# sharonct/CTPA-CLIP

Measured on AMD Instinct MI355X. Metric: CT-report pairs/sec (contrastive step), higher is better.
Workload: dtype bf16

## Files before the change

### ctpa-clip_amd/csrc/gemm256.hip

```cpp
#include "common.h"
#include <string.h>
#include "../../include/ctclip_hip.h"

namespace g256 {

constexpr int BN = 256, BK = 32;
constexpr int EP_LD = 68;
template <int WR> struct Cfg {
  static constexpr int BM = 128 * WR, NTH = 256 * WR;
  static constexpr int ABYTES = BM * BK * 2, BBYTES = BN * BK * 2, STAGE = ABYTES + BBYTES;
  static constexpr int NSTAGE = WR == 2 ? 4 : 3;
  static constexpr int SMEM = NSTAGE * STAGE;
  static constexpr int GA = ABYTES / 16 / NTH, GB = BBYTES / 16 / NTH, G = GA + GB;
};

struct P {
  int64_t M, N, K;
  const u16* A; int64_t lda;
  const u16* B; int64_t ldb;
  void* C; int64_t ldc; int c_f32;
  u16* C2; int64_t ldc2;
  const float* bias;
  const void* R; int64_t ldr; int r_f32;
  float alpha; int act; int accumulate; int split_k;
// ... 624 lines not shown
          bi = x > best ? c : bi;
          second = __builtin_amdgcn_fmed3f(best, second, x);
          best = fmaxf(best, x);
        }
      auto merge = [&](float ob, float os, int oi) {
        const bool take = ob > best || (ob == best && oi < bi);
        second = take ? fmaxf(best, os) : fmaxf(second, ob);
        bi = take ? oi : bi;
        best = take ? ob : best;
      };
      if (GEMM_PERMLANE) {
        { const float ob = xorf<16>(best, lane), os = xorf<16>(second, lane); merge(ob, os, xori<16>(bi, lane)); }
        { const float ob = xorf<32>(best, lane), os = xorf<32>(second, lane); merge(ob, os, xori<32>(bi, lane)); }
      } else {
#pragma unroll
        for (int o = 16; o <= 32; o <<= 1)
          merge(__shfl_xor(best, o, 64), __shfl_xor(second, o, 64), __shfl_xor(bi, o, 64));
      }
      if (g == 0 && rok && wcol0 < p.N) {
        float2* out = (float2*)p.C + bidx * p.sC;
        out[gm * p.ldc + (wcol0 >> 6)] = make_float2(best, __int_as_float((int)(wcol0 + bi)));
        if (p.C2) ((float*)p.C2)[bidx * p.sC2 + gm * p.ldc2 + (wcol0 >> 6)] = second;
      }
      continue;
    }
    if constexpr (MODE == 8) {
      if (fold) {
        const int64_t gr = rok ? gm : p.M - 1;
        const float mu = p.ln_mean[gr], rs = p.ln_rstd[gr];
#pragma unroll
        for (int j = 0; j < 4; ++j)
#pragma unroll
          for (int r = 0; r < 4; ++r) v[j][r] = rs * (v[j][r] - mu * bias[j][r]);
      }
    }
    if constexpr (MODE == 6 || MODE == 8) {
      float qb[4][4];
#pragma unroll
      for (int j = 0; j < 4; ++j)
#pragma unroll
        for (int r = 0; r < 4; ++r) qb[j][r] = bf2f(f2bf(v[j][r]));
      store_row_bf16((u16*)p.C + bidx * p.sC + gm * p.ldc + wcol0, v, g, rok && wcol0 >= p.c_col0, wcol0, p.N);
      if (wcol0 < p.n2) {
        const int d0 = pair_coff(g);
        const float* sp = p.bias + d0 + (MODE == 8 && !fold ? 32 : 0);
        const f32x4 s0v = *(const f32x4*)sp, s1v = *(const f32x4*)(sp + 4);
#pragma unroll
        for (int jp = 0; jp < 2; ++jp) {
          float c8[8];
#pragma unroll
          for (int k = 0; k < 4; ++k) {
            const auto r = __builtin_amdgcn_permlane16_swap(__float_as_uint(qb[2 * jp][k]),
                                                            __float_as_uint(qb[2 * jp + 1][k]), false, false);
            c8[k] = __uint_as_float(r[0]);
            c8[4 + k] = __uint_as_float(r[1]);
          }
          float ss = 0.f;
#pragma unroll
          for (int e = 0; e < 8; ++e) ss += c8[e] * c8[e];
          if (GEMM_PERMLANE) {
            ss += xorf<32>(ss, lane);
            ss += xorf<16>(ss, lane);
          } else {
            ss += __shfl_xor(ss, 32, 64);
            ss += __shfl_xor(ss, 16, 64);
          }
          const float inv = 1.f / fmaxf(sqrtf(ss), 1e-12f);
          float o8[8];
#pragma unroll
          for (int e = 0; e < 4; ++e) { o8[e] = c8[e] * inv * s0v[e]; o8[4 + e] = c8[4 + e] * inv * s1v[e]; }
          const int64_t c0 = wcol0 + 32 * jp + d0;
          if (rok && c0 < p.n2) st16(p.C2 + bidx * p.sC2 + gm * p.ldc2 + c0, pack8(o8));
        }
      }
      continue;
    }
    if constexpr (MODE == 5) {
      float* Cf = (float*)p.C + (int64_t)split * p.M * p.ldc + bidx * p.sC + gm * p.ldc + cl;
#pragma unroll
      for (int j = 0; j < 4; ++j)
        if (rok && cl + 16 * j < p.N) *(f32x4*)(Cf + 16 * j) = f32x4{v[j][0], v[j][1], v[j][2], v[j][3]};
      continue;
    }
    if constexpr (MODE == 2) {
      if constexpr (LDS) {
        const int64_t gm0 = wrow0 + i * 16;
        store_blk_bf16_lds(scr, (u16*)p.C + bidx * p.sC + gm0 * p.ldc + wcol0, p.ldc, gm0, p.M, wcol0, p.N, v, g, m,
                           lane, p.epi_lds == 2);
        float gg[2][4];
#pragma unroll
        for (int j = 0; j < 2; ++j)
#pragma unroll
          for (int r = 0; r < 4; ++r) gg[j][r] = gelu_erf(bf2f(f2bf(v[j + 2][r]))) * bf2f(f2bf(v[j][r]));
        *(u32x4*)(scr + SCR_GOFF + m * SCR_G + pair_coff(g) * 2) = pair_swap(gg[0], gg[1]);
        const int r = lane >> 2, c = (lane & 3) * 8;
        const u32x4 d = *(const u32x4*)(scr + SCR_GOFF + r * SCR_G + c * 2);
        if (gm0 + r < p.M && wcol0 < p.N) {
          if (p.epi_lds == 2) st16_sc1(p.C2 + bidx * p.sC2 + (gm0 + r) * p.ldc2 + (wcol0 >> 1) + c, d);
          else st16(p.C2 + bidx * p.sC2 + (gm0 + r) * p.ldc2 + (wcol0 >> 1) + c, d);
        }
        continue;
      }
      if constexpr (X3) {
        float gg[2][4], gh[2][4], gl[2][4], hv[4][4];
#pragma unroll
        for (int j = 0; j < 2; ++j)
#pragma unroll
          for (int r = 0; r < 4; ++r) {
            float ge, dge;
            gelu_erf_and_grad(v[j + 2][r], ge, dge);
            hv[j][r] = ge;
            hv[j + 2][r] = v[j][r] * dge;
            gg[j][r] = ge * v[j][r];
            gh[j][r] = rh(gg[j][r]);
            gl[j][r] = gg[j][r] - gh[j][r];
          }
        store_row_f16((u16*)p.C + bidx * p.sC + gm * p.ldc + wcol0, hv, g, rok, wcol0, p.N);
        const u32x4 dh = pair_swap_h(gh[0], gh[1]), dl = pair_swap_h(gl[0], gl[1]), db = pair_swap(gg[0], gg[1]);
        if (rok && wcol0 < p.N) {
          const int64_t gc = (wcol0 >> 1) + pair_coff(g);
          st16(p.C2 + bidx * p.sC2 + gm * p.ldc2 + gc, dh);
          st16(p.C3 + gm * p.ldc3 + gc, dl);
          if (p.C4) st16(p.C4 + gm * p.ldc4 + gc, db);
        }
        continue;
      }
      float gg[2][4];
      if constexpr (H16) {
        float hv[4][4];
#pragma unroll
        for (int j = 0; j < 2; ++j)
#pragma unroll
          for (int r = 0; r < 4; ++r) {
            const float xb = rh(v[j][r]);
            float ge, dge;
            gelu_erf_and_grad(rh(v[j + 2][r]), ge, dge);
            hv[j][r] = ge;
            hv[j + 2][r] = xb * dge;
            gg[j][r] = ge * xb;
          }
        store_row_f16((u16*)p.C + bidx * p.sC + gm * p.ldc + wcol0, hv, g, rok && p.C, wcol0, p.N);
      } else {
        store_row_bf16((u16*)p.C + bidx * p.sC + gm * p.ldc + wcol0, v, g, rok, wcol0, p.N, p.epi_lds == 3);
#pragma unroll
        for (int j = 0; j < 2; ++j)
#pragma unroll
          for (int r = 0; r < 4; ++r) gg[j][r] = gelu_erf(bf2f(f2bf(v[j + 2][r]))) * bf2f(f2bf(v[j][r]));
      }
      const u32x4 d = pair_swap(gg[0], gg[1]);
      if (rok && wcol0 < p.N) {
        if (p.epi_lds == 3) st16_sc1(p.C2 + bidx * p.sC2 + gm * p.ldc2 + (wcol0 >> 1) + pair_coff(g), d);
        else st16(p.C2 + bidx * p.sC2 + gm * p.ldc2 + (wcol0 >> 1) + pair_coff(g), d);
      }
      continue;
    }
    if constexpr (MODE != 0) continue;
#pragma unroll
    for (int j = 0; j < 4; ++j)
#pragma unroll
      for (int r = 0; r < 4; ++r) v[j][r] += bias[j][r];
    if (p.R) {
      if (p.r_f32) {
        const float* Rp = (const float*)p.R + bidx * p.sR + gm * p.ldr + cl;
#pragma unroll
        for (int j = 0; j < 4; ++j)
          if (rok && cl + 16 * j < p.N) {
            const f32x4 a = *(const f32x4*)(Rp + 16 * j);
#pragma unroll
            for (int r = 0; r < 4; ++r) v[j][r] += a[r];
          }
      } else {
        const u16* Rp = (const u16*)p.R + bidx * p.sR + gm * p.ldr + cl;
#pragma unroll
        for (int j = 0; j < 4; ++j)
          if (rok && cl + 16 * j < p.N) {
            float rr[4];
            unpack4(*(const uint2*)(Rp + 16 * j), rr);
#pragma unroll
            for (int r = 0; r < 4; ++r) v[j][r] += rr[r];
          }
      }
    }
    if (p.act == 1) {
      if (p.C2) store_row_bf16(p.C2 + bidx * p.sC2 + gm * p.ldc2 + wcol0, v, g, rok, wcol0, p.N);
#pragma unroll
      for (int j = 0; j < 4; ++j)
#pragma unroll
        for (int r = 0; r < 4; ++r) v[j][r] = gelu_erf(v[j][r]);
    }
    if (p.c_f32) {
      float* Cf = (float*)p.C + bidx * p.sC + gm * p.ldc + cl;
#pragma unroll
      for (int j = 0; j < 4; ++j)
        if (rok && cl + 16 * j < p.N) {
          if (p.accumulate) {
            const f32x4 a = *(const f32x4*)(Cf + 16 * j);
#pragma unroll
            for (int r = 0; r < 4; ++r) v[j][r] += a[r];
          }
          *(f32x4*)(Cf + 16 * j) = f32x4{v[j][0], v[j][1], v[j][2], v[j][3]};
        }
    } else {
      u16* Cb = (u16*)p.C + bidx * p.sC + gm * p.ldc + wcol0;
      if (p.accumulate) {
#pragma unroll
        for (int j = 0; j < 4; ++j)
          if (rok && cl + 16 * j < p.N) {
            float rr[4];
            unpack4(*(const uint2*)(Cb + 16 * j + 4 * g), rr);
#pragma unroll
            for (int r = 0; r < 4; ++r) v[j][r] += rr[r];
          }
      }
      if constexpr (LDS) {
        const int64_t gm0 = wrow0 + i * 16;
        store_blk_bf16_lds(scr, (u16*)p.C + bidx * p.sC + gm0 * p.ldc + wcol0, p.ldc, gm0, p.M, wcol0, p.N, v, g, m,
                           lane, p.epi_lds == 2);
      } else {
        store_row_bf16(Cb, v, g, rok, wcol0, p.N, p.epi_lds == 3);
      }
    }
    if (p.C2 && p.act == 0) {
      if constexpr (LDS) {
        const int64_t gm0 = wrow0 + i * 16;
        store_blk_bf16_lds(scr, p.C2 + bidx * p.sC2 + gm0 * p.ldc2 + wcol0, p.ldc2, gm0, p.M, wcol0, p.N, v, g, m,
                           lane, p.epi_lds == 2);
      } else {
        store_row_bf16(p.C2 + bidx * p.sC2 + gm * p.ldc2 + wcol0, v, g, rok, wcol0, p.N, p.epi_lds == 3);
      }
    }
  }
}

#ifndef GEGLU_BWD_LA
#define GEGLU_BWD_LA 1
#endif
__device__ __forceinline__ void epilogue_geglu_bwd(const P& p, f32x4 (&acc)[8][4], int wr, int wc, int lane,
                                                   int64_t m0, int64_t n0, int bidx) {
  const int m = lane & 15, g = lane >> 4;
  const int64_t wrow0 = m0 + wr * 128, wcol0 = n0 + wc * 64, t0 = wcol0 >> 5;
  const int co = pair_coff(g);
  const u16* hb = (const u16*)p.R + bidx * p.sR;
  u16* db = (u16*)p.C + bidx * p.sC;
  constexpr int LA = GEGLU_BWD_LA;
  u32x4 hx[LA + 1][2], hg[LA + 1][2];
  auto load = [&](int i, int b) {
    const int64_t gm = wrow0 + i * 16 + m;
#pragma unroll
    for (int jp = 0; jp < 2; ++jp) {
      const int64_t t = t0 + jp;
      if (gm < p.M && t * 32 < p.N) {
        const u16* hp = hb + gm * p.ldr + t * 64 + co;
        hx[b][jp] = *(const u32x4*)hp;
        hg[b][jp] = *(const u32x4*)(hp + 32);
      } else {
        hx[b][jp] = make_uint4(0, 0, 0, 0);
        hg[b][jp] = make_uint4(0, 0, 0, 0);
      }
    }
  };
#pragma unroll
  for (int i = 0; i < LA; ++i) load(i, i);
#pragma unroll
  for (int i = 0; i < 8; ++i) {
    const int b = i % (LA + 1);
    if (i + LA < 8) load(i + LA, (i + LA) % (LA + 1));
    const int64_t gm = wrow0 + i * 16 + m;
#pragma unroll
    for (int jp = 0; jp < 2; ++jp) {
      float v0[4], v1[4];
#pragma unroll
      for (int r = 0; r < 4; ++r) { v0[r] = acc[i][2 * jp][r] * p.alpha; v1[r] = acc[i][2 * jp + 1][r] * p.alpha; }
      float d[8], x[8], gt[8], ox[8], og[8];
      unpack8(pair_swap(v0, v1), d);
      if (p.h16) {
        unpack8h(hx[b][jp], x);
        unpack8h(hg[b][jp], gt);
#pragma unroll
        for (int k = 0; k < 8; ++k) {
          ox[k] = d[k] * x[k];
          og[k] = d[k] * gt[k];
        }
      } else {
        unpack8(hx[b][jp], x);
        unpack8(hg[b][jp], gt);
#pragma unroll
        for (int k = 0; k < 8; ++k) {
          float ge, dge;
          gelu_erf_and_grad(gt[k], ge, dge);
          ox[k] = d[k] * ge;
          og[k] = d[k] * x[k] * dge;
        }
      }
      const int64_t t = t0 + jp;
      if (gm < p.M && t * 32 < p.N) {
        u16* dp = db + gm * p.ldc + t * 64 + co;
        st16(dp, pack8(ox));
        st16(dp + 32, pack8(og));
      }
    }
  }
}

typedef __attribute__((address_space(1))) unsigned long long gu64;
typedef __attribute__((address_space(1))) int gi32;
constexpr int LN_ST = p8::SMEM_P;
constexpr int LN_FIN = LN_ST + 2 * 128 * 4 * 8;
constexpr int SMEM_LN = LN_FIN + 256 * 8;
constexpr unsigned LN_SPIN_LIMIT = 1u << 21;

__device__ __forceinline__ void chan(float& m, float& M2, float mb, float M2b, float half_n) {
  const float d = m - mb;
  M2 = (M2 + M2b) + d * d * half_n;
  m = 0.5f * (m + mb);
}

template <int MODE>
__device__ __forceinline__ void epilogue_ln(const P& p, f32x4 (&acc)[8][4], char* smem, int w, int wr, int wc,
                                            int lane, int64_t m0, int64_t n0) {
  float* cs = (float*)(smem + p8::TILEB + w * (32 * EP_LD * 4));
  float2* st = (float2*)(smem + LN_ST);
  float2* fin = (float2*)(smem + LN_FIN);
  const int tx = (int)(n0 >> 8);
  const int64_t wrow0 = m0 + wr * 128, wcol0 = n0 + wc * 64;
  const int cc = (lane & 7) * 8, rl = lane >> 3;
  const int64_t gn = wcol0 + cc;
  float gam[8], bet[8];
  {
    const f32x4 a = *(const f32x4*)(p.ln_gamma + gn), b = *(const f32x4*)(p.ln_gamma + gn + 4);
    f32x4 c = f32x4{0.f, 0.f, 0.f, 0.f}, d = c;
    if (MODE == 6 && p.ln_beta) { c = *(const f32x4*)(p.ln_beta + gn); d = *(const f32x4*)(p.ln_beta + gn + 4); }
#pragma unroll
    for (int j = 0; j < 4; ++j) { gam[j] = a[j]; gam[4 + j] = b[j]; bet[j] = c[j]; bet[4 + j] = d[j]; }
  }
  f32x4 b0 = f32x4{0.f, 0.f, 0.f, 0.f}, b1 = b0;
  if (MODE == 6 && p.bias) { b0 = *(const f32x4*)(p.bias + gn); b1 = *(const f32x4*)(p.bias + gn + 4); }
  float keep[4][4][8];
  float pg[8], pb[8];
#pragma unroll
  for (int j = 0; j < 8; ++j) { pg[j] = 0.f; pb[j] = 0.f; }

#pragma unroll
  for (int quarter = 0; quarter < 4; ++quarter) {
    __builtin_amdgcn_sched_barrier(0);
#pragma unroll
    for (int i = 0; i < 2; ++i)
#pragma unroll
      for (int j = 0; j < 4; ++j)
#pragma unroll
        for (int r = 0; r < 4; ++r)
          cs[(i * 16 + (lane >> 4) * 4 + r) * EP_LD + j * 16 + (lane & 15)] = acc[quarter * 2 + i][j][r];
    __builtin_amdgcn_s_waitcnt(0xC07F);
    const int64_t rbase = wrow0 + quarter * 32;
    if constexpr (MODE == 6) {
      f32x4 ra[4], rb[4];
#pragma unroll
      for (int it = 0; it < 4; ++it) {
        const float* Rp = (const float*)p.R + (rbase + it * 8 + rl) * p.ldr + gn;
        ra[it] = *(const f32x4*)Rp;
        rb[it] = *(const f32x4*)(Rp + 4);
      }
#pragma unroll
      for (int it = 0; it < 4; ++it) {
        const f32x4 lo = *(const f32x4*)(cs + (it * 8 + rl) * EP_LD + cc);
        const f32x4 hi = *(const f32x4*)(cs + (it * 8 + rl) * EP_LD + cc + 4);
#pragma unroll
        for (int j = 0; j < 4; ++j) {
          keep[quarter][it][j] = lo[j] * p.alpha + b0[j] + ra[it][j];
          keep[quarter][it][4 + j] = hi[j] * p.alpha + b1[j] + rb[it][j];
        }
      }
#pragma unroll
      for (int it = 0; it < 4; ++it) {
        const float* v = keep[quarter][it];
        float* Cf = (float*)p.C + (rbase + it * 8 + rl) * p.ldc + gn;
        *(f32x4*)Cf = f32x4{v[0], v[1], v[2], v[3]};
        *(f32x4*)(Cf + 4) = f32x4{v[4], v[5], v[6], v[7]};
      }
      if (p.C2) {
#pragma unroll
        for (int it = 0; it < 4; ++it) *(u32x4*)(p.C2 + (rbase + it * 8 + rl) * p.ldc2 + gn) = pack8(keep[quarter][it]);
      }
#pragma unroll
      for (int it = 0; it < 4; ++it) {
        const float* v = keep[quarter][it];
        float m = 0.f;
#pragma unroll
        for (int j = 0; j < 8; ++j) m += v[j];
        m *= 0.125f;
        float M2 = 0.f;
#pragma unroll
        for (int j = 0; j < 8; ++j) { const float d = v[j] - m; M2 += d * d; }
#pragma unroll
        for (int o = 1; o <= 4; o <<= 1) chan(m, M2, __shfl_xor(m, o, 64), __shfl_xor(M2, o, 64), 4.f * o);
        if ((lane & 7) == 0) st[(wr * 128 + quarter * 32 + it * 8 + rl) * 4 + wc] = make_float2(m, M2);
      }
    } else {
      float mu[4], rs[4];
      u32x4 kx[4];
#pragma unroll
      for (int it = 0; it < 4; ++it) {
        const int64_t row = rbase + it * 8 + rl;
        kx[it] = *(const u32x4*)(p.ln_x + row * p.ln_ldx + gn);
        mu[it] = p.ln_mean[row];
        rs[it] = p.ln_rstd[row];
      }
#pragma unroll
      for (int it = 0; it < 4; ++it) {
        const f32x4 lo = *(const f32x4*)(cs + (it * 8 + rl) * EP_LD + cc);
        const f32x4 hi = *(const f32x4*)(cs + (it * 8 + rl) * EP_LD + cc + 4);
        float d[8];
#pragma unroll
        for (int j = 0; j < 4; ++j) { d[j] = lo[j] * p.alpha; d[4 + j] = hi[j] * p.alpha; }
        const u32x4 kd = pack8(d);
        *(u32x4*)(p.C2 + (rbase + it * 8 + rl) * p.ldc2 + gn) = kd;
        float dy[8], xv[8];
        unpack8(kd, dy);
        unpack8(kx[it], xv);
        float s1 = 0.f, s2 = 0.f;
#pragma unroll
        for (int j = 0; j < 8; ++j) {
          const float xh = (xv[j] - mu[it]) * rs[it];
          const float g = dy[j] * gam[j];
          s1 += g;
          s2 += g * xh;
        }
#pragma unroll
        for (int o = 1; o <= 4; o <<= 1) { s1 += __shfl_xor(s1, o, 64); s2 += __shfl_xor(s2, o, 64); }
        if ((lane & 7) == 0) st[(wr * 128 + quarter * 32 + it * 8 + rl) * 4 + wc] = make_float2(s1, s2);
      }
    }
    __builtin_amdgcn_s_waitcnt(0xC07F);
  }
  __syncthreads();
  if (wc == 0) {
    gu64* X = (gu64*)p.xchg;
    const unsigned long long tag = (unsigned long long)p.epoch << 32;
    float a0[2], a1[2];
#pragma unroll
    for (int h = 0; h < 2; ++h) {
      const int r = lane + 64 * h;
      const float2 s0 = st[(wr * 128 + r) * 4 + 0], s1 = st[(wr * 128 + r) * 4 + 1];
      const float2 s2 = st[(wr * 128 + r) * 4 + 2], s3 = st[(wr * 128 + r) * 4 + 3];
      if constexpr (MODE == 6) {
        float m = s0.x, M2 = s0.y, mm = s2.x, MM = s2.y;
        chan(m, M2, s1.x, s1.y, 32.f);
        chan(mm, MM, s3.x, s3.y, 32.f);
        chan(m, M2, mm, MM, 64.f);
        a0[h] = m;
        a1[h] = M2;
      } else {
        a0[h] = (s0.x + s1.x) + (s2.x + s3.x);
        a1[h] = (s0.y + s1.y) + (s2.y + s3.y);
      }
      gu64* g = X + ((int64_t)tx * p.M + wrow0 + r) * 2;
      if (!(p.ln_debug && tx == 1 && m0 == 0)) {
        __hip_atomic_store(g, tag | __float_as_uint(a0[h]), __ATOMIC_RELAXED, __HIP_MEMORY_SCOPE_AGENT);
        __hip_atomic_store(g + 1, tag | __float_as_uint(a1[h]), __ATOMIC_RELAXED, __HIP_MEMORY_SCOPE_AGENT);
      }
    }
    const gu64* Y = X + (int64_t)(1 - tx) * p.M * 2;
    unsigned long long q[2][2];
    for (unsigned spins = 0;; ++spins) {
      bool ok = true;
#pragma unroll
      for (int h = 0; h < 2; ++h)
#pragma unroll
        for (int k = 0; k < 2; ++k) {
          q[h][k] = __hip_atomic_load(Y + (wrow0 + lane + 64 * h) * 2 + k, __ATOMIC_RELAXED, __HIP_MEMORY_SCOPE_AGENT);
          ok = ok && (unsigned)(q[h][k] >> 32) == p.epoch;
        }
      if (__all(ok)) break;
      if (spins >= p.spin_limit) {
        if (lane == 0 && p.status) __hip_atomic_store((gi32*)p.status, 1, __ATOMIC_RELAXED, __HIP_MEMORY_SCOPE_AGENT);
        break;
      }
      __builtin_amdgcn_s_sleep(1);
    }
#pragma unroll
    for (int h = 0; h < 2; ++h) {
      const int r = lane + 64 * h;
      const float o0 = __uint_as_float((unsigned)q[h][0]), o1 = __uint_as_float((unsigned)q[h][1]);
      float2 f;
      if constexpr (MODE == 6) {
        float m = a0[h], M2 = a1[h];
        chan(m, M2, o0, o1, 128.f);
        const float rstd = rsqrtf(M2 * (1.f / 512.f) + p.ln_eps);
        f = make_float2(m, rstd);
        if (tx == 0) {
          p.ln_mean[wrow0 + r] = m;
          p.ln_rstd[wrow0 + r] = rstd;
        }
      } else {
        f = make_float2((a0[h] + o0) * (1.f / 512.f), (a1[h] + o1) * (1.f / 512.f));
      }
      fin[wr * 128 + r] = f;
    }
  }
  __syncthreads();
  const u16* lx = p.ln_x;
  u16* lc2 = p.C2;
  const float* lmean = p.ln_mean;
  const float* lrstd = p.ln_rstd;
  int64_t frow0 = wrow0 + rl, fcol = gn;
  asm volatile("" : "+v"(frow0), "+v"(fcol));
#pragma unroll
  for (int quarter = 0; quarter < 4; ++quarter) {
    __builtin_amdgcn_sched_barrier(0);
    const int64_t rbase = frow0 - rl + quarter * 32;
    if constexpr (MODE == 6) {
#pragma unroll
      for (int it = 0; it < 4; ++it) {
        const float2 f = fin[wr * 128 + quarter * 32 + it * 8 + rl];
        float o[8];
#pragma unroll
        for (int j = 0; j < 8; ++j) o[j] = (keep[quarter][it][j] - f.x) * f.y * gam[j] + bet[j];
        if (p.ln_y) *(u32x4*)(p.ln_y + (rbase + it * 8 + rl) * p.ln_ldy + gn) = pack8(o);
        if (p.ln_y16) *(u32x4*)(p.ln_y16 + (rbase + it * 8 + rl) * p.ln_ldy + gn) = pack8h(o);
      }
    } else {
#pragma unroll
      for (int half = 0; half < 2; ++half) {
        __builtin_amdgcn_sched_barrier(0);
        f32x4 ra[2], rb[2];
        float mu[2], rs[2];
        u32x4 kx[2], kd[2];
        const int r0 = (int)frow0 + quarter * 32 + half * 16, c0 = (int)fcol;
#pragma unroll
        for (int it = 0; it < 2; ++it) {
          const int row = r0 + it * 8;
          kx[it] = *(const u32x4*)(lx + (row * (int)p.ln_ldx + c0));
          kd[it] = *(const u32x4*)(lc2 + (row * (int)p.ldc2 + c0));
          const float* Rp = (const float*)p.R + (row * (int)p.ldr + c0);
          ra[it] = *(const f32x4*)Rp;
          rb[it] = *(const f32x4*)(Rp + 4);
          mu[it] = lmean[row];
          rs[it] = lrstd[row];
        }
#pragma unroll
        for (int it = 0; it < 2; ++it) {
          const int row = r0 + it * 8;
          const float2 f = fin[wr * 128 + quarter * 32 + half * 16 + it * 8 + rl];
          float dy[8], xv[8], o[8];
          unpack8(kd[it], dy);
          unpack8(kx[it], xv);
#pragma unroll
          for (int j = 0; j < 8; ++j) {
            const float xh = (xv[j] - mu[it]) * rs[it];
            pg[j] += dy[j] * xh;
            pb[j] += dy[j];
            o[j] = rs[it] * (dy[j] * gam[j] - f.x - xh * f.y) + (j < 4 ? ra[it][j] : rb[it][j - 4]);
          }
          float* Cf = (float*)p.C + (row * (int)p.ldc + c0);
          *(f32x4*)Cf = f32x4{o[0], o[1], o[2], o[3]};
          *(f32x4*)(Cf + 4) = f32x4{o[4], o[5], o[6], o[7]};
          *(u32x4*)(lc2 + (row * (int)p.ldc2 + c0)) = pack8(o);
        }
      }
    }
  }
  if constexpr (MODE == 7) {
#pragma unroll
    for (int j = 0; j < 8; ++j)
#pragma unroll
      for (int o = 8; o <= 32; o <<= 1) { pg[j] += __shfl_xor(pg[j], o, 64); pb[j] += __shfl_xor(pb[j], o, 64); }
    if (rl == 0) {
      const int64_t slab = ((m0 >> 7) + wr) * p.N + gn;
      *(f32x4*)(p.ln_pg + slab) = f32x4{pg[0], pg[1], pg[2], pg[3]};
      *(f32x4*)(p.ln_pg + slab + 4) = f32x4{pg[4], pg[5], pg[6], pg[7]};
      if (p.ln_pb) {
        *(f32x4*)(p.ln_pb + slab) = f32x4{pb[0], pb[1], pb[2], pb[3]};
        *(f32x4*)(p.ln_pb + slab + 4) = f32x4{pb[4], pb[5], pb[6], pb[7]};
      }
    }
  }
}

struct Tile {
  int64_t m0, n0, kbeg;
  int nk, split, bidx;
};

template <bool X3 = false>
__device__ __forceinline__ Tile tile_at(const P& p, int lin, int gx, int gy, int ntiles) {
  int id = lin;
  if (ntiles >= 16) {
    const int xcd = lin & 7, q = ntiles >> 3, r = ntiles & 7;
    id = (xcd < r ? xcd * (q + 1) : r * (q + 1) + (xcd - r) * q) + (lin >> 3);
  }
  const int gxy = gx * gy, z = id / gxy, rem = id - z * gxy;
  int ty, tx;
  if (gx >= p.group_gx) {
    const int GM = p.group_gm > 0 ? p.group_gm : 8;
    const int grp = rem / (GM * gx), y0 = grp * GM, gsz = min(gy - y0, GM), r = rem - grp * GM * gx;
    ty = y0 + r % gsz;
    tx = r / gsz;
  } else {
    ty = rem / gx;
    tx = rem - ty * gx;
  }
  Tile t;
  t.split = z % p.split_k;
  t.bidx = z / p.split_k;
  t.m0 = (int64_t)ty * p8::BM;
  t.n0 = (int64_t)tx * p8::BNN;
  t.kbeg = t.split * p.kper;
  const int64_t kend = min(p.K, t.kbeg + p.kper);
  t.nk = (kend > t.kbeg && !(p.debug & 2)) ? (int)((kend - t.kbeg) / p8::BKK) * (X3 ? 3 : 1) : 0;
  return t;
}

#ifdef CTCLIP_GEMM_STAMPS
__device__ unsigned long long g_stamps[256][32][6];
#define STAMP(k, v)                                                                        \
  do {                                                                                     \
    const unsigned long long t_ = (v);                                                     \
    if (threadIdx.x == 0 && tcount < 32) g_stamps[blockIdx.x][tcount][k] = t_;             \
  } while (0)
#else
#define STAMP(k, v) do { } while (0)
#endif

template <bool AK, bool BKC, int EP, bool H16 = false, bool X3 = false>
__global__ __launch_bounds__(512, 1) void gemm8p_kernel(P p) {
  using namespace p8;
  constexpr bool TR = EP >= 0;
  extern __shared__ __attribute__((aligned(16))) char smem[];
  const int lane = threadIdx.x & 63, w = threadIdx.x >> 6, wr = w >> 2, wc = w & 3;
  const int gx = (int)((p.N + BNN - 1) / BNN), gy = (int)((p.M + BM - 1) / BM);
  const int ntiles = gx * gy * p.gz;
  int lin = p.persist ? (int)blockIdx.x : (int)((blockIdx.z * gridDim.y + blockIdx.y) * gridDim.x + blockIdx.x);
  const int lstride = p.persist ? (int)gridDim.x : ntiles;
  if (lin >= ntiles) return;
  Tile T = tile_at<X3>(p, lin, gx, gy, ntiles);
  if (p.stagger > 0 && lin < 256) {
    const int ng = p.stagger >= 1000 ? 4 : 2, u = p.stagger % 1000, grp = (lin >> 3) & (ng - 1);
    for (int s = 0; s < grp * u; ++s) __builtin_amdgcn_s_sleep(32);
  }

  f32x4 acc[8][4];
#pragma unroll
  for (int i = 0; i < 8; ++i)
#pragma unroll
    for (int j = 0; j < 4; ++j) acc[i][j] = f32x4{0.f, 0.f, 0.f, 0.f};
  const int wu = __builtin_amdgcn_readfirstlane(w);
  char* scr = smem + TILEB + (wu < 4 ? A1 : B1) * HALF + (wu & 3) * 4096;

  auto stage_of = [&](const Tile& tl, int which, int t) {
    if (t >= tl.nk) return;
    char* dst = smem + (t & 1) * TILEB + which * HALF;
    int tk = t;
    const u16* Ab = p.A;
    const u16* Bb = p.B;
    if constexpr (X3) {
      tk = (t * 21846) >> 16;
      const int sub = t - 3 * tk;
      if (sub == 2) Ab = p.alo;
      if (sub == 1) Bb = p.blo;
    }
    const int64_t k0 = tl.kbeg + (int64_t)tk * BKK;
    if (which < 2) stage_half<AK, true>(dst, Ab + tl.bidx * p.sA, p.lda, p.M, tl.m0, k0, which, w, lane);
    else stage_half<BKC, false>(dst, Bb + tl.bidx * p.sB, p.ldb, p.N, tl.n0, k0, which - 2, w, lane);
  };
  auto stage = [&](int which, int t) { stage_of(T, which, t); };

  bf16x8 a[4][2], b0[2][2], b1[2][2];

  const int abase = frag_base<AK>(wr * 64, lane), bbase = frag_base<BKC>(wc * 32, lane);
  auto load_frags = [&](int buf, int q) {
    const char* base = smem + buf * TILEB;
    if (q == 0 || q == 2) {
#pragma unroll
      for (int s = 0; s < 2; ++s)
#pragma unroll
        for (int ii = 0; ii < 4; ++ii) a[ii][s] = hfrag<AK>(base, q == 0 ? A0 : A1, abase, ii, s);
    }
    if (q == 0) {
#pragma unroll
      for (int s = 0; s < 2; ++s)
#pragma unroll
        for (int jj = 0; jj < 2; ++jj) b0[jj][s] = hfrag<BKC>(base, B0, bbase, jj, s);
    }
    if (q == 1) {
#pragma unroll
      for (int s = 0; s < 2; ++s)
#pragma unroll
        for (int jj = 0; jj < 2; ++jj) b1[jj][s] = hfrag<BKC>(base, B1, bbase, jj, s);
    }
  };
  auto mma = [&](int q) {
    const int mi = (q == 0 || q == 1) ? 0 : 1;
    const int ni = (q == 1 || q == 2) ? 1 : 0;
    __builtin_amdgcn_s_setprio(1);
#pragma unroll
    for (int s = 0; s < 2; ++s)
#pragma unroll
      for (int ii = 0; ii < 4; ++ii)
#pragma unroll
        for (int jj = 0; jj < 2; ++jj) {
          const bf16x8 bb = ni ? b1[jj][s] : b0[jj][s];
          acc[mi * 4 + ii][ni * 2 + jj] = TR ? mfma16<H16>(bb, a[ii][s], acc[mi * 4 + ii][ni * 2 + jj])
                                             : mfma16<H16>(a[ii][s], bb, acc[mi * 4 + ii][ni * 2 + jj]);
        }
    __builtin_amdgcn_s_setprio(0);
  };
  auto wait_ahead = [&](bool younger_issued) {
    if (younger_issued) asm volatile("s_waitcnt vmcnt(4)" ::: "memory");
    else asm volatile("s_waitcnt vmcnt(0)" ::: "memory");
  };
  auto compute_phase = [&]() {
    bar();
    asm volatile("s_waitcnt lgkmcnt(0)" ::: "memory");
    __builtin_amdgcn_sched_barrier(0);
  };

  stage(A0, 0); stage(A1, 0); stage(B0, 0); stage(B1, 0);
  stage(A0, 1); stage(B0, 1);
  wait_ahead(T.nk > 1);

  int tcount = 0;
  (void)tcount;
  constexpr bool PRE_OK = TR && (EP == 3 || EP == 4 || (EP == 0 && !BKC));
  bool pre = false;
  while (true) {
    const int nk = T.nk;
    STAMP(0, __builtin_amdgcn_s_memtime());
    STAMP(5, __builtin_amdgcn_s_memrealtime());
    bar();
    if (wr == 1) bar();
    for (int i = 0; 2 * i < nk; ++i) {
      if (i == 1) STAMP(2, __builtin_amdgcn_s_memtime());
      const int te = 2 * i, to = 2 * i + 1;
      const int t1 = (PRE_OK && i == 0 && pre) ? nk : to;
#pragma unroll
      for (int q = 0; q < 4; ++q) {
        load_frags(0, q);
        if (q == 0) stage(B1, t1);
        if (q == 1) stage(A1, t1);
        if (q == 2) stage(A0, te + 2);
        if (q == 3) { stage(B0, te + 2); if (to < nk) wait_ahead(te + 2 < nk); }
        compute_phase();
        mma(q);
        bar();
      }
      if (to < nk) {
#pragma unroll
        for (int q = 0; q < 4; ++q) {
          load_frags(1, q);
          if (q == 0) stage(B1, te + 2);
          if (q == 1) stage(A1, te + 2);
          if (q == 2) stage(A0, to + 2);
          if (q == 3) { stage(B0, to + 2); if (te + 2 < nk) wait_ahead(to + 2 < nk); }
          compute_phase();
          mma(q);
          bar();
        }
      }
    }
    if (wr == 0) bar();
    __syncthreads();
    STAMP(3, __builtin_amdgcn_s_memtime());
    lin += lstride;
    const bool more = lin < ntiles;
    if (more) {
      const Tile nx = tile_at<X3>(p, lin, gx, gy, ntiles);
      stage_of(nx, A0, 0); stage_of(nx, A1, 0); stage_of(nx, B0, 0); stage_of(nx, B1, 0);
      if constexpr (TR) { stage_of(nx, A0, 1); stage_of(nx, B0, 1); }
      if constexpr (PRE_OK) {
        if (p.pre1) { stage_of(nx, B1, 1); stage_of(nx, A1, 1); }
      }
    }
    pre = PRE_OK && more && p.pre1;
    if (p.debug & 1) {
#pragma unroll
      for (int i = 0; i < 8; ++i)
#pragma unroll
        for (int j = 0; j < 4; ++j) asm volatile("" ::"v"(acc[i][j]));
    } else if constexpr (EP == 2 || EP == 12) {
      epilogue_t<2, EP == 12, H16, X3>(p, acc, wr, wc, lane, T.m0, T.n0, T.split, T.bidx, scr);
    } else if constexpr (EP == 4) {
      epilogue_geglu_bwd(p, acc, wr, wc, lane, T.m0, T.n0, T.bidx);
    } else if constexpr (EP == 0 || EP == 10) {
      epilogue_t<0, EP == 10>(p, acc, wr, wc, lane, T.m0, T.n0, T.split, T.bidx, scr);
    } else if constexpr (EP == 3) {
      epilogue_t<3>(p, acc, wr, wc, lane, T.m0, T.n0, T.split, T.bidx, scr);
    } else if constexpr (EP == 6) {
      epilogue_t<6>(p, acc, wr, wc, lane, T.m0, T.n0, T.split, T.bidx, scr);
    } else if constexpr (EP == 8) {
      epilogue_t<8>(p, acc, wr, wc, lane, T.m0, T.n0, T.split, T.bidx, scr);
    } else if constexpr (EP == -8) {
      epilogue<-8>(p, acc, smem + TILEB, w, wr, wc, lane, T.m0, T.n0, T.split, T.bidx);
    } else if constexpr (EP == -6 || EP == -7) {
      epilogue_ln<EP == -6 ? 6 : 7>(p, acc, smem, w, wr, wc, lane, T.m0, T.n0);
    } else {
      epilogue<EP == -2 || EP == -3 || EP == -5 ? EP : -1>(p, acc, smem + TILEB, w, wr, wc, lane, T.m0, T.n0, T.split, T.bidx);
    }
    STAMP(4, __builtin_amdgcn_s_memtime());
    ++tcount;
    if (!more) break;
    T = tile_at<X3>(p, lin, gx, gy, ntiles);
#pragma unroll
    for (int i = 0; i < 8; ++i)
#pragma unroll
      for (int j = 0; j < 4; ++j) acc[i][j] = f32x4{0.f, 0.f, 0.f, 0.f};
    if constexpr (!TR) {
      __syncthreads();
      stage(A0, 1); stage(B0, 1);
    }
    wait_ahead(T.nk > 1);
  }
}

static int g_grid_cap = 0;

template <bool AK, bool BKC, int EP, bool H16 = false, bool X3 = false>
int launch8(const P& p, int batch, hipStream_t st) {
  constexpr int smem = EP == -6 || EP == -7 ? SMEM_LN : p8::SMEM_P;
  static bool attr = false;
  if (!attr) {
    (void)hipFuncSetAttribute((const void*)gemm8p_kernel<AK, BKC, EP, H16, X3>,
                              hipFuncAttributeMaxDynamicSharedMemorySize, smem);
    attr = true;
  }
  const int64_t ntiles = cdiv(p.N, p8::BNN) * cdiv(p.M, p8::BM) * (int64_t)p.gz;
  static bool cap_env = false;
  if (!cap_env) {
    const char* e = getenv("CTCLIP_GEMM_GRID_CAP");
    if (e && g_grid_cap == 0) g_grid_cap = atoi(e);
    cap_env = true;
  }
  static int pre1 = -1;
  if (pre1 < 0) { const char* e = getenv("CTCLIP_GEMM_PRE1"); pre1 = e ? atoi(e) != 0 : 1; }
  if (p.persist) {
    const int64_t cap = g_grid_cap > 0 && g_grid_cap < 256 ? g_grid_cap : 256;
    dim3 grid((unsigned)(ntiles < cap ? ntiles : cap));
    P q = p;
    q.pre1 = pre1;
    hipLaunchKernelGGL((gemm8p_kernel<AK, BKC, EP, H16, X3>), grid, dim3(p8::NTH), smem, st, q);
  } else {
    dim3 grid(cdiv(p.N, p8::BNN), cdiv(p.M, p8::BM), batch * p.split_k);
    hipLaunchKernelGGL((gemm8p_kernel<AK, BKC, EP, H16, X3>), grid, dim3(p8::NTH), smem, st, p);
  }
  CT_CHECK_LAUNCH();
  return 0;
}

template <int WR, bool AK, bool BKC>
int launch(const P& p, int batch, hipStream_t st) {
  using C = Cfg<WR>;
  static bool attr = false;
  if (!attr) {
    (void)hipFuncSetAttribute((const void*)gemm256_kernel<WR, AK, BKC>, hipFuncAttributeMaxDynamicSharedMemorySize,
                              C::SMEM);
    attr = true;
  }
  dim3 grid(cdiv(p.N, BN), cdiv(p.M, C::BM), batch * p.split_k);
  hipLaunchKernelGGL((gemm256_kernel<WR, AK, BKC>), grid, dim3(C::NTH), C::SMEM, st, p);
  CT_CHECK_LAUNCH();
  return 0;
}

template <int WR>
int launch_any(const P& p, bool ak, bool bk, int batch, hipStream_t st) {
  if (ak && bk) return launch<WR, true, true>(p, batch, st);
  if (ak) return launch<WR, true, false>(p, batch, st);
  if (bk) return launch<WR, false, true>(p, batch, st);
  return launch<WR, false, false>(p, batch, st);
}

static int g_variant = -1;
static int g_stagger8 = -1;
static int g_persist = -1;
static int g_epi_lds = -1;
int variant() {
  if (g_variant < 0) {
    const char* e = getenv("CTCLIP_GEMM_VARIANT");
    g_variant = e ? atoi(e) : 8;
    if (g_variant != 1 && g_variant != 2) g_variant = 8;
  }
  return g_variant;
}
int tile_rows() { return variant() == 2 ? 2 : 1; }

template <bool AK, bool BKC>
int launch8_ep(const P& p, int batch, hipStream_t st) {
  if (p.act == 4) return launch8<AK, BKC, 4>(p, batch, st);
  if (p.act == 5) return launch8<AK, BKC, 6>(p, batch, st);
  static int tr_f32 = -1;
  if (tr_f32 < 0) { const char* e = getenv("CTCLIP_GEMM_TR_F32"); tr_f32 = e ? atoi(e) != 0 : 0; }
  const bool tr = (tr_f32 || (!p.c_f32 && !p.R)) && p.split_k <= 1 && p.act != 3;
  if (!tr) {
    static int am_tr = -1;
    if (am_tr < 0) { const char* e = getenv("CTCLIP_GEMM_ARGMAX_TR"); am_tr = e ? atoi(e) != 0 : 1; }
    if (p.act == 3 && am_tr && p.split_k <= 1) return launch8<AK, BKC, 3>(p, batch, st);
    if (p.act == 3) return launch8<AK, BKC, -3>(p, batch, st);
    if (p.split_k > 1) return launch8<AK, BKC, -5>(p, batch, st);
    if (p.R && p.r_f32 && p.c_f32 && p.act == 0 && !p.accumulate) return launch8<AK, BKC, -2>(p, batch, st);
    return launch8<AK, BKC, -1>(p, batch, st);
  }
  const bool relay = p.epi_lds == 1 || p.epi_lds == 2;
  if (p.act == 2) return relay ? launch8<AK, BKC, 12>(p, batch, st) : launch8<AK, BKC, 2>(p, batch, st);
  return relay ? launch8<AK, BKC, 10>(p, batch, st) : launch8<AK, BKC, 0>(p, batch, st);
}

int launch8_h16(const P& p, int batch, hipStream_t st) {
  if (p.split_k > 1 || p.act == 4 || p.act == 5 || p.act == 6) return CT_EINVAL;
  if (p.act == 3) return p.x3 ? CT_EINVAL : launch8<true, true, 3, true>(p, batch, st);
  if (p.x3) {
    if (p.act == 2) return launch8<true, true, 2, true, true>(p, batch, st);
    if (!p.c_f32 || p.act != 0) return CT_EINVAL;
    if (p.R && p.r_f32 && !p.accumulate) return launch8<true, true, -2, true, true>(p, batch, st);
    if (p.R) return CT_EINVAL;
    return launch8<true, true, -1, true, true>(p, batch, st);
  }
  const bool tr = !p.c_f32 && !p.R;
  if (p.act == 2) return launch8<true, true, 2, true>(p, batch, st);
  if (tr) return launch8<true, true, 0, true>(p, batch, st);
  if (p.R && p.r_f32 && p.c_f32 && p.act == 0 && !p.accumulate) return launch8<true, true, -2, true>(p, batch, st);
  return launch8<true, true, -1, true>(p, batch, st);
}

template <bool AK>
int launch8_any(const P& p, bool bk, int batch, hipStream_t st) {
  return bk ? launch8_ep<AK, true>(p, batch, st) : launch8_ep<AK, false>(p, batch, st);
}

}

int ctclip_gemm256(const ctclip_gemm_args* a, int split, int batch, void* stream) {
  using namespace g256;
  P p{};
  memset(&p, 0, sizeof(p));
  p.M = a->M; p.N = a->N; p.K = a->K;
  p.A = (const u16*)a->A; p.lda = a->lda;
  p.B = (const u16*)a->B; p.ldb = a->ldb;
  p.C = a->C; p.ldc = a->ldc; p.c_f32 = a->c_f32;
  p.C2 = (u16*)a->C2; p.ldc2 = a->ldc2;
  p.bias = a->bias;
  p.R = a->R; p.ldr = a->ldr; p.r_f32 = a->r_f32;
  p.alpha = a->alpha; p.act = a->act; p.accumulate = a->accumulate; p.split_k = split;
  p.sA = a->sA; p.sB = a->sB; p.sC = a->sC; p.sC2 = a->sC2; p.sR = a->sR;
  p.n2 = a->n2;
  p.fold_cs = nullptr;
  p.nfold = 0;
  p.h16 = a->ab_f16 || a->r_f16;
  p.ln_y16 = nullptr;
  p.x3 = a->A_lo != nullptr;
  p.alo = (const u16*)a->A_lo;
  p.blo = (const u16*)a->B_lo;
  p.C3 = (u16*)a->C3; p.ldc3 = a->ldc3;
  p.C4 = (u16*)a->C4; p.ldc4 = a->ldc4;
  const int kstep = (variant() == 8 || a->act == 4 || a->act == 5) ? p8::BKK : BK;
  p.kper = (a->K / kstep + split - 1) / split * kstep;
  static int dbg = -1, stag = 0;
  if (dbg < 0) {
    const char* e = getenv("CTCLIP_G256_DEBUG");
    dbg = e ? atoi(e) : 0;
    const char* s = getenv("CTCLIP_G256_STAGGER");
    stag = s ? atoi(s) : 0;
  }
  p.debug = dbg;
  if (g_persist < 0) {
    const char* e = getenv("CTCLIP_GEMM_PERSIST");
    g_persist = e ? (atoi(e) != 0) : 1;
  }
  p.gz = batch * split;
  p.persist = g_persist;
  if (g_epi_lds < 0) {
    const char* e = getenv("CTCLIP_EPI_LDS");
    g_epi_lds = e ? std::min(3, std::max(0, atoi(e))) : 0;
  }
  p.epi_lds = g_epi_lds;
  static int ggx = -1;
  if (ggx < 0) { const char* e = getenv("CTCLIP_GEMM_GROUP_GX"); ggx = e ? atoi(e) : 8; }
  p.group_gx = ggx;
  static int ggm = -1;
  if (ggm < 0) { const char* e = getenv("CTCLIP_GEMM_GROUP_GM"); ggm = e ? atoi(e) : 8; }
  p.group_gm = ggm;
  p.stagger = variant() == 8 ? (g_stagger8 >= 0 ? g_stagger8 : (a->act == 4 ? 8 : 0)) : (tile_rows() == 1 ? stag : 0);
  hipStream_t st = (hipStream_t)stream;
  if (a->ab_f16) {
    if (!a->a_kcontig || !a->b_kcontig) return CT_EINVAL;
    p.stagger = 0;
    return launch8_h16(p, batch, st);
  }
  if (variant() == 8 || a->act == 4 || a->act == 5)
    return a->a_kcontig ? launch8_any<true>(p, a->b_kcontig, batch, st) : launch8_any<false>(p, a->b_kcontig, batch, st);
  if (tile_rows() == 2) return launch_any<2>(p, a->a_kcontig, a->b_kcontig, batch, st);
  return launch_any<1>(p, a->a_kcontig, a->b_kcontig, batch, st);
}

extern "C" int ctclip_gemm_ln(const ctclip_gemm_args* a, const ctclip_ln_epilogue* ln, void* stream) {
  using namespace g256;
  if (!a || !ln || (ln->mode != 1 && ln->mode != 2)) return CT_EINVAL;
  if (a->M == 0) return 0;
  CT_REQUIRE(a->N == 512 && a->M > 0 && a->M % 2048 == 0 && a->K > 0 && a->K % 64 == 0, CT_ESHAPE);
  CT_REQUIRE(a->split_k <= 1 && a->batch <= 1 && a->act == 0 && !a->accumulate && a->c_f32 && !a->B2, CT_EINVAL);
  CT_REQUIRE(variant() == 8 && g_persist != 0 && g_grid_cap == 0, CT_EINVAL);
  CT_REQUIRE(aligned16(a->A) && aligned16(a->B) && aligned16(a->C) && a->lda % 8 == 0 && a->ldb % 8 == 0 &&
                 a->ldc % 8 == 0, CT_EALIGN);
  if (a->C2) CT_REQUIRE(aligned16(a->C2) && a->ldc2 % 8 == 0, CT_EALIGN);
  if (a->R) CT_REQUIRE(a->r_f32 && aligned16(a->R) && a->ldr % 8 == 0, CT_EINVAL);
  if (a->bias) CT_REQUIRE(ln->mode == 1 && aligned16(a->bias), CT_EINVAL);
  CT_REQUIRE(ln->gamma && aligned16(ln->gamma) && ln->mean && ln->rstd && ln->xchg && ln->epoch != 0 &&
                 (((uintptr_t)ln->xchg) & 7) == 0, CT_EINVAL);
  {
    const int64_t ldmax = std::max(std::max(a->ldc, a->ldc2), std::max(a->ldr, ln->ldx));
    CT_REQUIRE(a->M * ldmax < ((int64_t)1 << 31), CT_ESHAPE);
  }
  if (ln->mode == 1) {
    CT_REQUIRE(a->R && (ln->Y || ln->Y16) && aligned16(ln->Y) && aligned16(ln->Y16) && ln->ldy % 8 == 0, CT_EINVAL);
    if (ln->beta) CT_REQUIRE(aligned16(ln->beta), CT_EALIGN);
  } else {
    CT_REQUIRE(ln->X && aligned16(ln->X) && ln->ldx % 8 == 0 && ln->part_gamma && !ln->beta && a->C2 && a->R,
               CT_EINVAL);
  }
  P p{};
  memset(&p, 0, sizeof(p));
  p.M = a->M; p.N = a->N; p.K = a->K;
  p.A = (const u16*)a->A; p.lda = a->lda;
  p.B = (const u16*)a->B; p.ldb = a->ldb;
  p.C = a->C; p.ldc = a->ldc; p.c_f32 = 1;
  p.C2 = (u16*)a->C2; p.ldc2 = a->ldc2;
  p.bias = a->bias;
  p.R = a->R; p.ldr = a->ldr; p.r_f32 = 1;
  p.alpha = a->alpha; p.act = 0; p.accumulate = 0; p.split_k = 1;
  p.kper = a->K;
  p.debug = 0;
  p.group_gx = 1 << 30;
  p.stagger = 0;
  p.gz = 1;
  p.persist = 1;
  p.ln_gamma = ln->gamma; p.ln_beta = ln->beta; p.ln_eps = ln->eps;
  p.ln_y = (u16*)ln->Y; p.ln_ldy = ln->ldy;
  p.ln_mean = ln->mean; p.ln_rstd = ln->rstd;
  p.ln_x = (const u16*)ln->X; p.ln_ldx = ln->ldx;
  p.ln_pg = ln->part_gamma; p.ln_pb = ln->part_beta;
  p.xchg = (unsigned long long*)ln->xchg;
  p.epoch = ln->epoch;
  p.status = ln->status;
  p.spin_limit = ln->spin_limit ? ln->spin_limit : LN_SPIN_LIMIT;
  p.ln_debug = ln->debug;
  p.ln_y16 = ln->mode == 1 ? (u16*)ln->Y16 : nullptr;
  hipStream_t st = (hipStream_t)stream;
  if (!a->a_kcontig) return CT_EINVAL;
  if (a->ab_f16) {
    if (ln->mode != 1 || !a->b_kcontig) return CT_EINVAL;
    return launch8<true, true, -6, true>(p, 1, st);
  }
  if (ln->mode == 1) return a->b_kcontig ? launch8<true, true, -6>(p, 1, st) : launch8<true, false, -6>(p, 1, st);
  return a->b_kcontig ? launch8<true, true, -7>(p, 1, st) : launch8<true, false, -7>(p, 1, st);
}

extern "C" int ctclip_gemm_qkv_lnfold(const ctclip_gemm_args* a, const float* mean, const float* rstd,
                                      const float* fold_cs, int32_t nfold, void* stream) {
  return ctclip_gemm_qkv_lnfold2(a, mean, rstd, fold_cs, nfold, 0, stream);
}

extern "C" int ctclip_gemm_qkv_lnfold2(const ctclip_gemm_args* a, const float* mean, const float* rstd,
                                       const float* fold_cs, int32_t nfold, int32_t c_col0, void* stream) {
  using namespace g256;
  if (c_col0 < 0 || c_col0 % 64) return CT_EINVAL;
  if (!a || !mean || !rstd || !fold_cs) return CT_EINVAL;
  if (a->M == 0) return 0;
  CT_REQUIRE(a->M > 0 && a->N % 256 == 0 && a->K > 0 && a->K % 64 == 0, CT_ESHAPE);
  CT_REQUIRE(nfold > 0 && nfold % 256 == 0 && nfold < a->N && a->n2 > nfold && a->n2 % 64 == 0 && a->n2 <= a->N,
             CT_EINVAL);
  CT_REQUIRE(a->a_kcontig && a->b_kcontig && !a->c_f32 && a->C2 && a->bias && !a->R && !a->B2 && a->act == 5 &&
                 a->split_k <= 1 && a->batch <= 1 && !a->accumulate,
             CT_EINVAL);
  CT_REQUIRE(variant() == 8, CT_EINVAL);
  CT_REQUIRE(aligned16(a->A) && aligned16(a->B) && aligned16(a->C) && aligned16(a->C2) && aligned16(a->bias) &&
                 aligned16(fold_cs) && a->lda % 8 == 0 && a->ldb % 8 == 0 && a->ldc % 8 == 0 && a->ldc2 % 8 == 0,
             CT_EALIGN);
  P p{};
  memset(&p, 0, sizeof(p));
  p.M = a->M; p.N = a->N; p.K = a->K;
  p.A = (const u16*)a->A; p.lda = a->lda;
  p.B = (const u16*)a->B; p.ldb = a->ldb;
  p.C = a->C; p.ldc = a->ldc; p.c_f32 = 0;
  p.C2 = (u16*)a->C2; p.ldc2 = a->ldc2;
  p.bias = a->bias;
  p.alpha = a->alpha; p.act = 5; p.split_k = 1;
  p.n2 = a->n2;
  p.kper = a->K;
  p.gz = 1;
  if (g_persist < 0) {
    const char* e = getenv("CTCLIP_GEMM_PERSIST");
    g_persist = e ? (atoi(e) != 0) : 1;
  }
  p.persist = g_persist;
  p.group_gx = 8;
  p.ln_mean = (float*)mean;
  p.ln_rstd = (float*)rstd;
  p.fold_cs = fold_cs;
  p.nfold = nfold;
  p.c_col0 = c_col0;
  if (a->ab_f16) return launch8<true, true, 8, true>(p, 1, (hipStream_t)stream);
  return launch8<true, true, 8>(p, 1, (hipStream_t)stream);
}

extern "C" int ctclip_gemm_lnfold_bwd(const ctclip_gemm_args* a, const void* X, int64_t ldx, const float* c1,
                                      const float* beta, void* stream) {
  using namespace g256;
  if (!a || !X || !c1 || !beta) return CT_EINVAL;
  if (a->M == 0) return 0;
  CT_REQUIRE(a->M > 0 && a->N > 0 && a->N % 8 == 0 && a->K > 0 && a->K % 64 == 0, CT_ESHAPE);
  CT_REQUIRE(a->a_kcontig && a->c_f32 && a->R && a->r_f32 && !a->bias && !a->B2 && a->act == 0 && a->split_k <= 1 &&
                 a->batch <= 1 && !a->accumulate,
             CT_EINVAL);
  CT_REQUIRE(variant() == 8, CT_EINVAL);
  CT_REQUIRE(aligned16(a->A) && aligned16(a->B) && aligned16(a->C) && aligned16(a->R) && aligned16(X) &&
                 a->lda % 8 == 0 && a->ldb % 8 == 0 && a->ldc % 8 == 0 && a->ldr % 8 == 0 && ldx % 8 == 0,
             CT_EALIGN);
  if (a->C2) CT_REQUIRE(aligned16(a->C2) && a->ldc2 % 8 == 0, CT_EALIGN);
  P p{};
  memset(&p, 0, sizeof(p));
  p.M = a->M; p.N = a->N; p.K = a->K;
  p.A = (const u16*)a->A; p.lda = a->lda;
  p.B = (const u16*)a->B; p.ldb = a->ldb;
  p.C = a->C; p.ldc = a->ldc; p.c_f32 = 1;
  p.C2 = (u16*)a->C2; p.ldc2 = a->ldc2;
  p.R = a->R; p.ldr = a->ldr; p.r_f32 = 1;
  p.alpha = a->alpha; p.split_k = 1;
  p.kper = a->K;
  p.gz = 1;
  if (g_persist < 0) {
    const char* e = getenv("CTCLIP_GEMM_PERSIST");
    g_persist = e ? (atoi(e) != 0) : 1;
  }
  p.persist = g_persist;
  p.group_gx = 8;
  p.ln_x = (const u16*)X;
  p.ln_ldx = ldx;
  p.ln_mean = (float*)c1;
  p.ln_rstd = (float*)beta;
  hipStream_t st = (hipStream_t)stream;
  return a->b_kcontig ? launch8<true, true, -8>(p, 1, st) : launch8<true, false, -8>(p, 1, st);
}

extern "C" int ctclip_gemm_set_epi_lds(int v) {
  const int old = g256::g_epi_lds;
  g256::g_epi_lds = v >= 0 && v <= 3 ? v : 0;
  return old;
}

extern "C" int ctclip_gemm_set_stagger(int v) {
  const int old = g256::g_stagger8;
  g256::g_stagger8 = v;
  return old;
}

extern "C" int ctclip_gemm_set_grid_cap(int v) {
  const int old = g256::g_grid_cap;
  g256::g_grid_cap = v > 0 ? v : 0;
  return old;
}

extern "C" int ctclip_gemm_set_persist(int v) {
  const int old = g256::g_persist;
  g256::g_persist = v != 0;
  return old;
}

extern "C" int ctclip_gemm_set_variant(int v) {
  const int old = g256::variant();
  if (v == 1 || v == 2 || v == 8) g256::g_variant = v;
  return old;
}

#ifdef CTCLIP_GEMM_STAMPS
extern "C" int ctclip_gemm_stamps(void* host, int clear) {
  hipError_t e = hipMemcpyFromSymbol(host, HIP_SYMBOL(g256::g_stamps), sizeof(g256::g_stamps), 0, hipMemcpyDeviceToHost);
  if (e == hipSuccess && clear) {
    static unsigned long long zero[256 * 32 * 6];
    e = hipMemcpyToSymbol(HIP_SYMBOL(g256::g_stamps), zero, sizeof(zero), 0, hipMemcpyHostToDevice);
  }
  return (int)e;
}
#endif
```

Measured before the change: 205.9.

## Relay GEGLU backward epilogue through LDS for coalesced row loads and stores

Result: faster. 208.3, median of 6 (+1.2%).

```diff
diff --git a/ctpa-clip_amd/csrc/gemm256.hip b/ctpa-clip_amd/csrc/gemm256.hip
--- a/ctpa-clip_amd/csrc/gemm256.hip
+++ b/ctpa-clip_amd/csrc/gemm256.hip
@@ -950,6 +950,84 @@
   }
 }
 
+#ifndef GEGLU_BWD_ROWS_LA
+#define GEGLU_BWD_ROWS_LA 1
+#endif
+constexpr int GB_STRIP = 16 * 256;
+constexpr int SMEM_GB = 2 * p8::TILEB + 8 * GB_STRIP;
+__device__ __forceinline__ void epilogue_geglu_bwd_rows(const P& p, f32x4 (&acc)[8][4], int wr, int wc, int lane,
+                                                        int64_t m0, int64_t n0, int bidx, char* scr) {
+  const int64_t wrow0 = m0 + wr * 128, wcol0 = n0 + wc * 64, t0 = wcol0 >> 5;
+  if (wcol0 >= p.N) return;
+  asm volatile("" : "+v"(lane));
+  const int m = lane & 15, g = lane >> 4;
+  const int rr = lane >> 4, pc = lane & 15;
+  const bool cok = (t0 + (pc >> 3)) * 32 < p.N;
+  const u16* hb = (const u16*)p.R + bidx * p.sR + t0 * 64 + pc * 8;
+  u16* db = (u16*)p.C + bidx * p.sC + t0 * 64 + pc * 8;
+  const int cx = pair_coff(g) >> 3;
+  constexpr int LA = GEGLU_BWD_ROWS_LA;
+  u32x4 hr[LA][4];
+  auto load = [&](int i, int b) {
+#pragma unroll
+    for (int q = 0; q < 4; ++q) {
+      const int64_t gm = wrow0 + i * 16 + q * 4 + rr;
+      hr[b][q] = (gm < p.M && cok) ? *(const u32x4*)(hb + gm * p.ldr) : make_uint4(0, 0, 0, 0);
+    }
+  };
+#pragma unroll
+  for (int i = 0; i < LA; ++i) load(i, i);
+#pragma unroll
+  for (int i = 0; i < 8; ++i) {
+    const int b = i % LA;
+#pragma unroll
+    for (int q = 0; q < 4; ++q) {
+      const int r = q * 4 + rr;
+      *(u32x4*)(scr + r * 256 + ((pc ^ r) << 4)) = hr[b][q];
+    }
+    if (i + LA < 8) load(i + LA, b);
+#pragma unroll
+    for (int jp = 0; jp < 2; ++jp) {
+      char* sx = scr + m * 256 + (((jp * 8 + cx) ^ m) << 4);
+      char* sg = scr + m * 256 + (((jp * 8 + 4 + cx) ^ m) << 4);
+      const u32x4 hx = *(const u32x4*)sx, hg = *(const u32x4*)sg;
+      float v0[4], v1[4];
+#pragma unroll
+      for (int r = 0; r < 4; ++r) { v0[r] = acc[i][2 * jp][r] * p.alpha; v1[r] = acc[i][2 * jp + 1][r] * p.alpha; }
+      float d[8], x[8], gt[8], ox[8], og[8];
+      unpack8(pair_swap(v0, v1), d);
+      if (p.h16) {
+        unpack8h(hx, x);
+        unpack8h(hg, gt);
+#pragma unroll
+        for (int k = 0; k < 8; ++k) {
+          ox[k] = d[k] * x[k];
+          og[k] = d[k] * gt[k];
+        }
+      } else {
+        unpack8(hx, x);
+        unpack8(hg, gt);
+#pragma unroll
+        for (int k = 0; k < 8; ++k) {
+          float ge, dge;
+          gelu_erf_and_grad(gt[k], ge, dge);
+          ox[k] = d[k] * ge;
+          og[k] = d[k] * x[k] * dge;
+        }
+      }
+      *(u32x4*)sx = pack8(ox);
+      *(u32x4*)sg = pack8(og);
+    }
+#pragma unroll
+    for (int q = 0; q < 4; ++q) {
+      const int r = q * 4 + rr;
+      const int64_t gm = wrow0 + i * 16 + r;
+      const u32x4 dv = *(const u32x4*)(scr + r * 256 + ((pc ^ r) << 4));
+      if (gm < p.M && cok) st16(db + gm * p.ldc, dv);
+    }
+  }
+}
+
 typedef __attribute__((address_space(1))) unsigned long long gu64;
 typedef __attribute__((address_space(1))) int gi32;
 constexpr int LN_ST = p8::SMEM_P;
@@ -1368,7 +1446,7 @@
 
   int tcount = 0;
   (void)tcount;
-  constexpr bool PRE_OK = TR && (EP == 3 || EP == 4 || (EP == 0 && !BKC));
+  constexpr bool PRE_OK = TR && (EP == 3 || EP == 4 || EP == 14 || (EP == 0 && !BKC));
   bool pre = false;
   while (true) {
     const int nk = T.nk;
@@ -1428,6 +1506,8 @@
       epilogue_t<2, EP == 12, H16, X3>(p, acc, wr, wc, lane, T.m0, T.n0, T.split, T.bidx, scr);
     } else if constexpr (EP == 4) {
       epilogue_geglu_bwd(p, acc, wr, wc, lane, T.m0, T.n0, T.bidx);
+    } else if constexpr (EP == 14) {
+      epilogue_geglu_bwd_rows(p, acc, wr, wc, lane, T.m0, T.n0, T.bidx, smem + 2 * TILEB + wu * GB_STRIP);
     } else if constexpr (EP == 0 || EP == 10) {
       epilogue_t<0, EP == 10>(p, acc, wr, wc, lane, T.m0, T.n0, T.split, T.bidx, scr);
     } else if constexpr (EP == 3) {
@@ -1463,7 +1543,7 @@
 
 template <bool AK, bool BKC, int EP, bool H16 = false, bool X3 = false>
 int launch8(const P& p, int batch, hipStream_t st) {
-  constexpr int smem = EP == -6 || EP == -7 ? SMEM_LN : p8::SMEM_P;
+  constexpr int smem = EP == -6 || EP == -7 ? SMEM_LN : EP == 14 ? SMEM_GB : p8::SMEM_P;
   static bool attr = false;
   if (!attr) {
     (void)hipFuncSetAttribute((const void*)gemm8p_kernel<AK, BKC, EP, H16, X3>,
@@ -1532,7 +1612,11 @@
 
 template <bool AK, bool BKC>
 int launch8_ep(const P& p, int batch, hipStream_t st) {
-  if (p.act == 4) return launch8<AK, BKC, 4>(p, batch, st);
+  if (p.act == 4) {
+    static int gb_rows = -1;
+    if (gb_rows < 0) { const char* e = getenv("CTCLIP_GEGLU_BWD_RELAY"); gb_rows = e ? atoi(e) != 0 : 1; }
+    return gb_rows ? launch8<AK, BKC, 14>(p, batch, st) : launch8<AK, BKC, 4>(p, batch, st);
+  }
   if (p.act == 5) return launch8<AK, BKC, 6>(p, batch, st);
   static int tr_f32 = -1;
   if (tr_f32 < 0) { const char* e = getenv("CTCLIP_GEMM_TR_F32"); tr_f32 = e ? atoi(e) != 0 : 0; }
```
